# NVIDIA/flowtron

Hardware: AMD Instinct MI355X
Metric: mel-frames/sec training (2-flow, 80-mel) (higher is better)
Workload: dtype bf16; 1 GPU; BASELINE configs[1]: 2-flow LJS config.json model, per-GPU batch 32, T_max=862, L_max=157, attn-prior + CTC on, fwd+loss+bwd+clip+RAdam; global_batch=32, parallelism=dp1, mfma_operands=bf16, storage=fp32, skipped_steps=0

## Files before the change

flowtron_amd/_lib.py:

```python
from __future__ import annotations

import ctypes as C
import os

import torch

_HERE = os.path.dirname(os.path.abspath(__file__))
LIB_PATH = os.path.join(_HERE, "libflowtron_hip.so")

FT_F32, FT_BF16, FT_F16 = 0, 1, 2
GEMM_SPLITK = 1
GEMM_SPLITK_DET = 2
GEMM_C16 = 4
ACT_NONE, ACT_TANH, ACT_RELU, ACT_SIGMOID = 0, 1, 2, 3

_p, _i, _l, _f, _sz, _d = C.c_void_p, C.c_int, C.c_int64, C.c_float, C.c_size_t, C.c_double


class GemmArgs(C.Structure):
    _fields_ = [("A", _p), ("B", _p), ("C", _p), ("bias", _p),
                ("M", _i), ("N", _i), ("K", _i), ("batch", _i),
                ("sAm", _l), ("sAk", _l), ("sBk", _l), ("sBn", _l), ("ldc", _l),
                ("bsA", _l), ("bsB", _l), ("bsC", _l),
                ("alpha", _f), ("beta", _f), ("act", _i), ("mode", _i), ("flags", _i),
                ("work", _p), ("work_bytes", _sz)]


class GemmImgArgs(C.Structure):
    _fields_ = [("A", _p), ("B", _p), ("C", _p), ("bias", _p), ("M", _i), ("N", _i), ("K", _i),
                ("lda", _l), ("ldb", _l), ("ldc", _l), ("a_kmajor", _i), ("b_kmajor", _i),
                ("alpha", _f), ("beta", _f), ("act", _i), ("flags", _i),
                ("rowmap", _p), ("rows_dev", _p), ("compact", _i), ("k_shift", _i), ("r1_row", _p), ("r1_col", _p),
                ("split_work", _p), ("split_work_bytes", _sz), ("a_rows", _p)]


class GemmImgPlan(C.Structure):
    _fields_ = [(n, _i) for n in ("tile_rows", "stage_k", "gather", "atomics", "det", "splits", "chunk_w")]


class GemmImgGroupPlan(C.Structure):
    _fields_ = [(n, _i) for n in ("tile_rows", "splits", "ksteps", "atomics", "launch", "unit0", "tiles")]


GEMM_GROUP_MAX = 48


class LstmFwdRole(C.Structure):
    _fields_ = [("gx", _p), ("lens", _p), ("y", _p), ("ldy", _l), ("gates", _p), ("cell", _p), ("wimg", _p), ("state_h", _p), ("state_c", _p),
                ("B", C.c_int32), ("ldb", C.c_int32), ("t0", C.c_int32), ("t1", C.c_int32), ("gx16", C.c_int32)]


class LstmBwdRole(C.Structure):
# ... 34 lines not shown
STYLE_BATCH, STYLE_TIME_AND_BATCH = 0, 1

SIGNATURES = {
    "ft_abi_version": ([], _i),
    "ft_last_error": ([], C.c_char_p),
    "ft_debug_hold_cus": ([_i, _l, _p], _i),
    "ft_gemm": ([C.POINTER(GemmArgs), _p], _i),
    "ft_gemm_workspace_bytes": ([C.POINTER(GemmArgs)], _sz),
    "ft_bf16_image_bytes": ([_l, _l], _sz),
    "ft_bf16_image": ([_p, _l, _l, _l, _p, _p], _i),
    "ft_bf16_image_colsum": ([_p, _l, _l, _l, _p, _p, _p], _i),
    "ft_bf16_image_colsum_acc": ([_p, _l, _l, _l, _p, _p, _p], _i),
    "ft_gemm_img": ([C.POINTER(GemmImgArgs), _p], _i),
    "ft_gemm_img_split_work_bytes": ([_i, _i, _i], _sz),
    "ft_gemm_img_plan": ([C.POINTER(GemmImgArgs), C.POINTER(GemmImgPlan)], _i),
    "ft_gemm_img_group": ([C.POINTER(GemmImgArgs), _i, _p], _i),
    "ft_gemm_img_group_plan": ([C.POINTER(GemmImgArgs), _i, C.POINTER(GemmImgGroupPlan)], _i),
    "ft_bf16_image_split3": ([_p, _l, _l, _l, _p, _i, _p], _i),
    "ft_bf16_image_split3_im2col": ([_p, _p, _i, _i, _i, _i, _p, _p], _i),
    "ft_bf16_image_split3_im2col_f16": ([_p, _p, _i, _i, _i, _i, _p, _p], _i),
    "ft_bf16_image_table": ([C.POINTER(ImgDesc), _i, _p], _i),
    "ft_bf16_image_table_f16": ([C.POINTER(ImgDesc), _i, _p], _i),
    "ft_bf16_image_split3_f16": ([_p, _l, _l, _l, _p, _i, _p], _i),
    "ft_rowmap_build": ([_p, _p, _p, _i, _i, _p], _i),
    "ft_chunk_gather_rows": ([_p, _p, _p, _i, _i, _i, _i, _p], _i),
    "ft_bf16_image_rows": ([_p, _l, _l, _l, _p, _p, _p, _p, _p], _i),
    "ft_bf16_image_rows_acc": ([_p, _l, _l, _l, _p, _p, _p, _p, _p], _i),
    "ft_bf16_image_rows_into": ([_p, _l, _l, _l, _p, _l, _l, _l, _p, _p, _p], _i),
    "ft_img_gemv_rows": ([_p, _l, _i, _p, _p, _p, _l, _p, _p, _p, _i, _i, _p], _i),
    "ft_img_gemv_rows_bwd": ([_p, _l, _i, _p, _l, _p, _p, _p, _p, _l, _p], _i),
# ... 207 lines not shown
```

flowtron_amd/csrc/api.hip:

```cpp
#include "common.h"

thread_local char g_ft_err[512] = {0};

extern "C" int ft_abi_version(void) { return FT_ABI_VERSION; }
extern "C" const char* ft_last_error(void) { return g_ft_err; }

namespace {
__global__ __launch_bounds__(64) void hold_cus_k(long long ticks, int* sink) {
    extern __shared__ int big[];
    const long long t0 = wall_clock64();
    int n = 0;
    while (wall_clock64() - t0 < ticks) { big[threadIdx.x] = ++n; __builtin_amdgcn_s_sleep(64); }
    if (sink && big[threadIdx.x] == -1) sink[0] = n;
}
}
extern "C" int ft_debug_hold_cus(int n_wg, int64_t ticks, void* stream) {
    FT_CHECK_ARG(n_wg >= 1 && n_wg <= 256 && ticks >= 0);
    if (ticks > 500000000LL) ticks = 500000000LL;
    const int lds = 160 * 1024;
    FT_CHECK_HIP(hipFuncSetAttribute(reinterpret_cast<const void*>(hold_cus_k), hipFuncAttributeMaxDynamicSharedMemorySize, lds));
    hipLaunchKernelGGL(hold_cus_k, dim3(n_wg), dim3(64), lds, reinterpret_cast<hipStream_t>(stream), (long long)ticks, (int*)nullptr);
    FT_CHECK_LAUNCH();
    return FT_OK;
}
// ... 1 lines not shown
```

flowtron_amd/csrc/common.h:

```cpp
#pragma once
#include <hip/hip_runtime.h>
#include <stdint.h>
#include <stdio.h>
#include <stdarg.h>
#include "../../include/flowtron_hip.h"

extern thread_local char g_ft_err[512];

static inline int ft_fail(int code, const char* fmt, ...) {
    va_list ap;
    va_start(ap, fmt);
    vsnprintf(g_ft_err, sizeof(g_ft_err), fmt, ap);
    va_end(ap);
    return code;
}

#define FT_CHECK_ARG(cond)                                                            \
    do {                                                                              \
        if (!(cond)) return ft_fail(FT_EINVAL, "%s: invalid argument: %s", __func__, #cond); \
    } while (0)

#define FT_CHECK_LAUNCH()                                                             \
    do {                                                                              \
        hipError_t e_ = hipGetLastError();                                            \
// ... 137 lines not shown
```

flowtron_amd/csrc/gemm_bf16.hip:

```cpp
#include "common.h"
#include <stdlib.h>

namespace {

constexpr int TB = 128;

inline size_t up(size_t v, size_t m) { return (v + m - 1) / m * m; }

__device__ __forceinline__ uint4 pack8(const float (&v)[8]) {
    uint4 o;
    o.x = pack_op16x2(v[0], v[1]); o.y = pack_op16x2(v[2], v[3]);
    o.z = pack_op16x2(v[4], v[5]); o.w = pack_op16x2(v[6], v[7]);
    return o;
}

__device__ __forceinline__ int mapped_rows(const int* rdev, int Rp, int& Rz) {
    const int R = *rdev;
    const int z = (R + 32 + 255) & ~255;
    Rz = z < Rp ? z : Rp;
    return R;
}

__device__ __forceinline__ void img_rows_body(const float* __restrict__ src, long sr, long sc, int R, int Cc,
                                              unsigned short* __restrict__ dst, int Rp, int Cp, int vec,
// ... 182 lines not shown
}

struct BfP {
    const unsigned short* A; const unsigned short* B; float* C; const float* bias;
    int M, N, nk;
    long lda, ldb, ldc;
    float alpha, beta;
    int act, gx, gy, splits, ksteps;
    int vec_c;
    const int* rowmap; const int* rows_dev; int compact, k_shift;
    int chunk_w;
    const float* r1row; const float* r1col;
    long c_slice;
    int c16;
    const int* a_rows;
};

typedef __attribute__((address_space(3))) void lds_void;
typedef const __attribute__((address_space(1))) void glb_void;
typedef __attribute__((ext_vector_type(4))) short bf16x4;

template <bool KM, int RT = 128>
struct Operand {
    static constexpr int NS = RT / 64;
    static constexpr int WT = RT / 32;
    const unsigned short* src[NS];
    size_t kstride;
    int dst[NS];
    int roff;
    __device__ __forceinline__ void init(const unsigned short* img, long ld, int r0, int wave, int lane, int wsel) {
        const int li = lane & 15, kg = lane >> 4;
// ... 86 lines not shown
    }
    __device__ __forceinline__ void issue(unsigned char* sbuf, int t) const {
#pragma unroll
        for (int g = 0; g < NS; ++g) {
            if constexpr (GA)
                __builtin_amdgcn_global_load_lds((glb_void*)(srcg[g] + (size_t)t * 64), (lds_void*)(sbuf + dst0 + g * 1024), 16, 0, 0);
            else
                __builtin_amdgcn_global_load_lds((glb_void*)(src0 + (size_t)t * 64 + (size_t)g * ld8 + ((g & 1) ? xodd : 0)),
                                                 (lds_void*)(sbuf + dst0 + g * 1024), 16, 0, 0);
        }
    }
    __device__ __forceinline__ bf16x8 frag(const unsigned char* sbuf, int i, int ks) const {
        return *reinterpret_cast<const bf16x8*>(sbuf + ((roff + (i << 11)) ^ (ks << 6)));
    }
};

template <bool AKM, bool BKM, bool SPLIT, int RTA, int KS = 32, bool SB = false, bool GA = false>
__device__ __forceinline__ void gemm_bf16_body(const BfP& p, int tile, const int slice, const int nslices, const bool plain) {
    static_assert(!SB || (KS == 64 && RTA == 128 && !SPLIT), "single-buffer form: 128 x 128 x 64 store kernels");
    static_assert(!GA || (SB && !AKM), "row gather: the single-buffer form, k-contiguous A");
    constexpr int KQ = KS / 32;
    constexpr int OPA = RTA * 64 * KQ, OPB = 8192 * KQ;
    constexpr int TI = RTA / 32;
    __shared__ __attribute__((aligned(1024))) unsigned char smem[(SB ? 1 : 2) * (OPA + OPB)];
    const int tid = threadIdx.x, lane = tid & 63, wave = tid >> 6;
    const int wm = wave >> 1, wn = wave & 1;
    const int li = lane & 15, kg = lane >> 4;
    int t0 = slice * p.ksteps;
    int t1 = (t0 + p.ksteps < p.nk) ? t0 + p.ksteps : p.nk;
    int rows_lim = p.M, gy = p.gy;
// ... 2 lines not shown
        if (p.compact == 1) {
            rows_lim = R < p.M ? R : p.M;
            gy = (rows_lim + RTA - 1) / RTA;
            if (gy == 0) return;
        } else {
            int nk_eff = (R - p.k_shift + 31) >> 5;
            nk_eff = nk_eff < p.nk ? nk_eff : p.nk;
            if constexpr (SPLIT) {
                const int ks = (nk_eff + nslices - 1) / nslices;
                t0 = slice * ks;
                t1 = t0 + ks < nk_eff ? t0 + ks : nk_eff;
                if (t0 >= t1) return;
            } else t1 = t1 < nk_eff ? t1 : nk_eff;
        }
    }
    int mt, nt;
    if (p.chunk_w > 0 && gy >= 16) {
        const int xcd = tile & 7, idx = tile >> 3;
        const int qm = gy >> 3, rm = gy & 7;
        const int mh = qm + (xcd < rm ? 1 : 0);
        const int m_lo = xcd * qm + (xcd < rm ? xcd : rm);
        if (idx >= mh * p.gx) return;
        const int per_chunk = mh * p.chunk_w;
        const int ch = idx / per_chunk, within = idx - ch * per_chunk;
        const int left = p.gx - ch * p.chunk_w;
        const int cw = left < p.chunk_w ? left : p.chunk_w;
        const int mi = within / cw;
        mt = m_lo + mi;
        nt = ch * p.chunk_w + (within - mi * cw);
    } else {
        const int total = p.gx * gy, q = total >> 3, r = total & 7;
        const int xcd = tile & 7, idx = tile >> 3;
        if (tile >= total) return;
        tile = xcd * q + (xcd < r ? xcd : r) + idx;
        mt = tile / p.gx;
        nt = tile % p.gx;
    }
    const int m0 = mt * RTA, n0 = nt * TB;

    Operand<AKM, RTA> oa;
    Operand<BKM, 128> ob;
    Operand64<RTA, GA> oa64;
    Operand64<128> ob64;
    if constexpr (GA) oa64.init_rows(p.A, p.lda, m0, wave, lane, wm, p.a_rows, rows_lim - 1);
    else if constexpr (KS == 64 && !AKM) oa64.init(p.A, p.lda, m0, wave, lane, wm); else oa.init(p.A, p.lda, m0, wave, lane, wm);
    if constexpr (KS == 64 && !BKM) ob64.init(p.B, p.ldb, n0, wave, lane, wn); else ob.init(p.B, p.ldb, n0, wave, lane, wn);

    f32x4 acc[TI][4];
// ... 37 lines not shown
        }
        if constexpr (BKM) {
#pragma unroll
            for (int j = 0; j < 4; ++j) b[j] = __builtin_shufflevector(tb[2 * j], tb[2 * j + 1], 0, 1, 2, 3, 4, 5, 6, 7);
        }
    };
    auto multiply = [&](const bf16x8 (&a)[TI], const bf16x8 (&b)[4]) {
#pragma unroll
        for (int i = 0; i < TI; ++i)
#pragma unroll
            for (int j = 0; j < 4; ++j) {
                if constexpr (SPLIT) acc[i][j] = mfma16(a[i], b[j], acc[i][j]);
                else acc[i][j] = mfma16(b[j], a[i], acc[i][j]);
            }
    };
    const int s0 = t0 / KQ, s1 = (t1 + KQ - 1) / KQ;
    if (s0 < s1) issue_stage(smem, s0);
    if constexpr (SB) {
        for (int t = s0; t < s1; ++t) {
            asm volatile("s_waitcnt vmcnt(0)" ::: "memory");
            __syncthreads();
            bf16x8 a0[TI], b0[4], a1[TI], b1[4];
            load_frags(smem, 0, a0, b0);
            multiply(a0, b0);
            load_frags(smem, 1, a1, b1);
            __syncthreads();
            if (t + 1 < s1) issue_stage(smem, t + 1);
            multiply(a1, b1);
        }
    } else {
        for (int t = s0; t < s1; ++t) {
// ... 20 lines not shown
                if (p.compact == 1) { row = p.rowmap[row]; if (row < 0) continue; }
#pragma unroll
                for (int j = 0; j < 4; ++j) {
                    const int col = n0 + wn * 64 + j * 16 + li;
                    if (col >= p.N) continue;
                    float v = p.alpha * acc[i][j][r];
                    if (p.bias && slice == 0) v += p.bias[col];
                    float* cp = p.C + (long)row * p.ldc + col;
                    if (plain) *cp = p.beta != 0.f ? *cp + v : v;
                    else atomicAdd(cp, v);
                }
            }
        return;
    }

    const bool vec = p.vec_c != 0;
#pragma unroll
    for (int i = 0; i < TI; ++i) {
        int row = m0 + wm * (RTA / 2) + i * 16 + li;
        if (row >= rows_lim) continue;
        if (p.compact == 1) { row = p.rowmap[row]; if (row < 0) continue; }
#pragma unroll
        for (int j = 0; j < 4; ++j) {
            const int col = n0 + wn * 64 + j * 16 + kg * 4;
            if (col >= p.N) continue;
            float* cp = p.C + (size_t)slice * p.c_slice + (long)row * p.ldc + col;
            float v[4] = {p.alpha * acc[i][j][0], p.alpha * acc[i][j][1], p.alpha * acc[i][j][2], p.alpha * acc[i][j][3]};
            const int nv = (p.N - col < 4) ? p.N - col : 4;
            const bool full = vec && nv == 4;
            if (p.beta != 0.f) {
                if (full) { const float4 c = *reinterpret_cast<const float4*>(cp); v[0] += p.beta * c.x; v[1] += p.beta * c.y; v[2] += p.beta * c.z; v[3] += p.beta * c.w; }
                else for (int r = 0; r < nv; ++r) v[r] += p.beta * cp[r];
            }
            const float r1 = p.r1row ? p.r1row[row] : 0.f;
#pragma unroll
            for (int r = 0; r < 4; ++r) {
                if (r < nv && p.bias) v[r] += p.bias[col + r];
                if (r < nv && p.r1row) v[r] = fmaf(r1, p.r1col[col + r], v[r]);
                if (p.act == FT_ACT_TANH) v[r] = tanhf_(v[r]);
                else if (p.act == FT_ACT_RELU) v[r] = fmaxf(v[r], 0.f);
                else if (p.act == FT_ACT_SIGMOID) v[r] = sigmoidf_(v[r]);
            }
            if (p.c16) {
                unsigned short* hp = reinterpret_cast<unsigned short*>(p.C) + (long)row * p.ldc + col;
                if (full) *reinterpret_cast<uint2*>(hp) = make_uint2(pack_op16x2(v[0], v[1]), pack_op16x2(v[2], v[3]));
                else for (int r = 0; r < nv; ++r) hp[r] = f2op16(v[r]);
            } else if (full) *reinterpret_cast<float4*>(cp) = make_float4(v[0], v[1], v[2], v[3]);
            else for (int r = 0; r < nv; ++r) cp[r] = v[r];
        }
    }
}

template <bool AKM, bool BKM, bool SPLIT, int RTA, int KS = 32, bool SB = false, bool GA = false>
__global__ __launch_bounds__(256, SB ? 4 : (RTA == 256 || KS == 64) ? 2 : 4) void gemm_bf16_k(BfP p) {
    gemm_bf16_body<AKM, BKM, SPLIT, RTA, KS, SB, GA>(p, blockIdx.x, blockIdx.y, gridDim.y, false);
}

constexpr int GROUP_MAX = 48;
constexpr int GROUP_PLAIN = 1 << 8, GROUP_BETA1 = 1 << 9, GROUP_COMPACT = 1 << 10, GROUP_SHIFT = 12;
struct GroupTable {
    const unsigned short* A[GROUP_MAX]; const unsigned short* B[GROUP_MAX]; float* C[GROUP_MAX]; const float* bias[GROUP_MAX];
    const int* rows_dev[GROUP_MAX];
    float alpha[GROUP_MAX];
    int M[GROUP_MAX], N[GROUP_MAX], nk[GROUP_MAX], lda[GROUP_MAX], ldb[GROUP_MAX], ldc[GROUP_MAX];
    int how[GROUP_MAX];
// ... 10 lines not shown
        const int mid = (d + hi) >> 1;
        if (u >= t.unit0[mid]) d = mid; else hi = mid;
    }
    const int how = t.how[d], splits = how & 0xff;
    BfP p;
    p.A = t.A[d]; p.B = t.B[d]; p.C = t.C[d]; p.bias = t.bias[d];
    p.M = t.M[d]; p.N = t.N[d]; p.nk = t.nk[d];
    p.lda = t.lda[d]; p.ldb = t.ldb[d]; p.ldc = t.ldc[d];
    p.alpha = t.alpha[d]; p.beta = (how & GROUP_BETA1) ? 1.f : 0.f;
    p.act = FT_ACT_NONE;
    p.gx = (p.N + TB - 1) / TB; p.gy = (p.M + RTA - 1) / RTA;
    p.splits = splits; p.ksteps = (p.nk + splits - 1) / splits;
    p.vec_c = 0;
    p.rowmap = nullptr; p.rows_dev = t.rows_dev[d]; p.compact = (how & GROUP_COMPACT) ? 2 : 0; p.k_shift = how >> GROUP_SHIFT;
    p.chunk_w = 0; p.r1row = nullptr; p.r1col = nullptr; p.c_slice = 0; p.c16 = 0; p.a_rows = nullptr;
    const int local = u - t.unit0[d], tiles = p.gx * p.gy;
    const int slice = local / tiles;
    gemm_bf16_body<true, true, true, RTA>(p, local - slice * tiles, slice, splits, (how & GROUP_PLAIN) != 0);
}


struct KernelSel { int tile_rows, stage_k, gather, atomics; };

template <bool AKM, bool BKM>
void launch_s(const BfP& p, dim3 grid, const KernelSel& k, hipStream_t st) {
    if (k.tile_rows == 256) {
        if (k.atomics) hipLaunchKernelGGL((gemm_bf16_k<AKM, BKM, true, 256>), grid, dim3(256), 0, st, p);
        else hipLaunchKernelGGL((gemm_bf16_k<AKM, BKM, false, 256>), grid, dim3(256), 0, st, p);
    } else {
        if (k.atomics) hipLaunchKernelGGL((gemm_bf16_k<AKM, BKM, true, 128>), grid, dim3(256), 0, st, p);
        else if constexpr (!(AKM && BKM)) {
            if constexpr (!AKM) {
                if (k.gather) { hipLaunchKernelGGL((gemm_bf16_k<false, BKM, false, 128, 64, true, true>), grid, dim3(256), 0, st, p); return; }
            }
            if (k.stage_k == 64) hipLaunchKernelGGL((gemm_bf16_k<AKM, BKM, false, 128, 64, true>), grid, dim3(256), 0, st, p);
            else hipLaunchKernelGGL((gemm_bf16_k<AKM, BKM, false, 128>), grid, dim3(256), 0, st, p);
        } else hipLaunchKernelGGL((gemm_bf16_k<AKM, BKM, false, 128>), grid, dim3(256), 0, st, p);
    }
}

__global__ __launch_bounds__(256) void splitk_reduce_k(const float* __restrict__ work, int S, long MN, int N, float* __restrict__ C, long ldc,
                                                       const float* __restrict__ bias) {
    const long n4 = MN >> 2;
    for (long i = blockIdx.x * (long)blockDim.x + threadIdx.x; i < n4; i += (long)gridDim.x * blockDim.x) {
        const long e = i << 2;
        const long m = e / N;
        const int n = (int)(e - m * N);
        float4 a = *reinterpret_cast<const float4*>(work + e);
        for (int sl = 1; sl < S; ++sl) {
            const float4 b = *reinterpret_cast<const float4*>(work + (size_t)sl * MN + e);
            a.x += b.x; a.y += b.y; a.z += b.z; a.w += b.w;
        }
        if (bias) { a.x += bias[n]; a.y += bias[n + 1]; a.z += bias[n + 2]; a.w += bias[n + 3]; }
        *reinterpret_cast<float4*>(C + m * ldc + n) = a;
// ... 15 lines not shown
        const long smax = K / 512;
        if (s > smax) s = smax;
        if (s > 64) s = 64;
        if (s < 1) s = 1;
    }
    if (compact == 1) s = 1;
    *big_out = big;
    return s;
}

struct ImgPlan {
    bool big, wide, det_on;
    bool atomics;
    KernelSel sel;
    int gx, gy, ksteps, splits, chunk_w, gridx, vec_c, c16;
};
int plan_images(const float* C, long ldc, int a_km, int b_km, int M, int N, int K, float beta, int act, int flags, int compact, bool r1,
                const void* split_work, size_t split_work_bytes, bool a_rows, ImgPlan* pl) {
    pl->c16 = (flags & FT_GEMM_C16) ? 1 : 0;
    if (pl->c16 && (beta != 0.f || (flags & (FT_GEMM_SPLITK | FT_GEMM_SPLITK_DET))))
        return ft_fail(FT_EINVAL, "ft_gemm_img: FT_GEMM_C16 takes beta == 0 and no split-K");
    const bool det = (flags & FT_GEMM_SPLITK_DET) && split_work && act == FT_ACT_NONE && beta == 0.f && compact == 0 && !r1 && K >= 2048 &&
                     N % 4 == 0 && ldc % 4 == 0 && reinterpret_cast<uintptr_t>(C) % 16 == 0 && reinterpret_cast<uintptr_t>(split_work) % 16 == 0;
    const bool can_split = det || ((flags & FT_GEMM_SPLITK) && act == FT_ACT_NONE && (beta == 0.f || beta == 1.f) && K >= 2048 && !r1);
    bool big;
    long s = plan_slices(M, N, K, can_split, compact, &big);
    const int RTA = big ? 256 : TB;
    const int nk = cdiv(K, 32);
    pl->big = big;
    pl->gx = cdiv(N, TB); pl->gy = cdiv(M, RTA);
// ... 11 lines not shown
    if (a_rows && (!pl->wide || pl->splits != 1))
        return ft_fail(FT_EINVAL, "ft_gemm_img: a_rows is read by the 64-wide single-buffer kernel only (FT_GEMM_BF16_WIDE=0 / FT_GEMM_BF16_TILE=256 exclude it)");
    pl->det_on = det && pl->splits > 1;
    pl->atomics = pl->splits > 1 && !pl->det_on;
    pl->sel.tile_rows = big ? 256 : TB;
    pl->sel.atomics = pl->atomics ? 1 : 0;
    pl->sel.stage_k = (pl->wide && !pl->atomics) ? 64 : 32;
    pl->sel.gather = (a_rows && pl->sel.stage_k == 64) ? 1 : 0;
    static const int order_on = [] { const char* e = getenv("FT_GEMM_BF16_ORDER"); return e ? atoi(e) : 1; }();
    pl->chunk_w = 0;
    pl->gridx = pl->gx * pl->gy;
    if (order_on && pl->splits == 1 && pl->gy >= 16) {
        long cw = (2l << 20) / ((long)TB * (long)nk * 32 * 2);
        pl->chunk_w = (int)(cw < 1 ? 1 : (cw > pl->gx ? pl->gx : cw));
        pl->gridx = 8 * ((pl->gy + 7) / 8) * pl->gx;
    }
    return FT_OK;
}

int run_images(const unsigned short* A, long lda, int a_km, const unsigned short* B, long ldb, int b_km, float* C, long ldc,
               const float* bias, int M, int N, int K, float alpha, float beta, int act, int flags, hipStream_t st,
               const int* rowmap = nullptr, const int* rows_dev = nullptr, int compact = 0, int k_shift = 0,
               const float* r1row = nullptr, const float* r1col = nullptr, float* split_work = nullptr, size_t split_work_bytes = 0,
               const int* a_rows = nullptr) {
    ImgPlan pl;
    const int prc = plan_images(C, ldc, a_km, b_km, M, N, K, beta, act, flags, compact, r1row != nullptr, split_work, split_work_bytes,
                                a_rows != nullptr, &pl);
    if (prc != FT_OK) return prc;
    BfP p;
    p.a_rows = a_rows;
// ... 1 lines not shown
    p.M = M; p.N = N; p.nk = cdiv(K, 32); p.lda = lda; p.ldb = ldb; p.ldc = ldc;
    p.alpha = alpha; p.beta = beta; p.act = act;
    p.rowmap = rowmap; p.rows_dev = rows_dev; p.compact = compact; p.k_shift = k_shift;
    p.r1row = r1row; p.r1col = r1col;
    p.c_slice = 0;
    p.c16 = pl.c16;
    p.gx = pl.gx; p.gy = pl.gy; p.vec_c = pl.vec_c;
    p.ksteps = pl.ksteps; p.splits = pl.splits; p.chunk_w = pl.chunk_w;
    const bool det_on = pl.det_on;
    if (det_on) {
        p.C = split_work; p.ldc = N; p.c_slice = (long)M * N; p.bias = nullptr;
        p.vec_c = 1;
    } else if (p.splits > 1 && beta == 0.f) {
        FT_CHECK_HIP(hipMemset2DAsync(C, sizeof(float) * ldc, 0, sizeof(float) * N, M, st));
    }
    const dim3 grid(pl.gridx, p.splits);
    if (a_km) { if (b_km) launch_s<true, true>(p, grid, pl.sel, st); else launch_s<true, false>(p, grid, pl.sel, st); }
    else      { if (b_km) launch_s<false, true>(p, grid, pl.sel, st); else launch_s<false, false>(p, grid, pl.sel, st); }
    if (det_on) {
        const long n4 = ((long)M * N) >> 2;
        const int blocks = (int)((n4 + 255) / 256 < 4096 ? (n4 + 255) / 256 : 4096);
        hipLaunchKernelGGL(splitk_reduce_k, dim3(blocks), dim3(256), 0, st, split_work, p.splits, (long)M * N, N, C, ldc, bias);
    }
    FT_CHECK_LAUNCH();
    return FT_OK;
}

#define IMG_CHECK_ARG(cond)                                                           \
    do {                                                                              \
        if (!(cond)) return ft_fail(FT_EINVAL, "%s: invalid argument: %s", who, #cond); \
    } while (0)
// ... 344 lines not shown
    if (const int rc = check_img_args(a, __func__)) return rc;
    FT_CHECK_ARG(out != nullptr);
    ImgPlan pl;
    const int rc = plan_images(a->C, a->ldc, a->a_kmajor, a->b_kmajor, a->M, a->N, a->K, a->beta, a->act, a->flags, a->compact,
                               a->r1_row != nullptr, a->split_work, a->split_work_bytes, a->a_rows != nullptr, &pl);
    if (rc != FT_OK) return rc;
    out->tile_rows = pl.sel.tile_rows;
    out->stage_k = pl.sel.stage_k;
    out->gather = pl.sel.gather;
    out->atomics = pl.sel.atomics;
    out->det = pl.det_on ? 1 : 0;
    out->splits = pl.splits;
    out->chunk_w = pl.chunk_w;
    return FT_OK;
}
#endif

extern "C" int FT_OPNAME(ft_gemm_img)(const ft_gemm_img_args* a, void* stream) {
    if (const int rc = check_img_args(a, __func__)) return rc;
    return run_images(reinterpret_cast<const unsigned short*>(a->A), a->lda, a->a_kmajor, reinterpret_cast<const unsigned short*>(a->B),
                      a->ldb, a->b_kmajor, a->C, a->ldc, a->bias, a->M, a->N, a->K, a->alpha, a->beta, a->act, a->flags,
                      reinterpret_cast<hipStream_t>(stream), a->rowmap, a->rows_dev, a->compact, a->k_shift, a->r1_row, a->r1_col,
                      reinterpret_cast<float*>(a->split_work), a->split_work_bytes, a->a_rows);
}

#if FT_OPFMT == 0
extern "C" int ft_gemm_img_group_plan(const ft_gemm_img_args* probs, int n, ft_gemm_img_group_plan_t* out) {
    FT_CHECK_ARG(out != nullptr);
    GroupProb g[GROUP_MAX];
    int order[2][GROUP_MAX], cnt[2];
// ... 104 lines not shown
```

flowtron_amd/ops.py:

```python
from __future__ import annotations

import ctypes as C
from typing import List, Optional, Sequence

import torch

from . import _lib as L



def _c(t: torch.Tensor) -> torch.Tensor:
    return t if t.is_contiguous() else t.contiguous()


import os as _os
_BF16_IMAGES = True


def gemm_raw(A, B, Cm, M, N, K, sAm, sAk, sBk, sBn, ldc, bias=None, act=L.ACT_NONE, alpha=1.0, beta=0.0,
             batch=1, bsA=0, bsB=0, bsC=0, mode=None, splitk=False):
    L.require_cuda(A, B, Cm, bias)
    a = L.GemmArgs(L.ptr(A), L.ptr(B), L.ptr(Cm), L.ptr(bias), M, N, K, batch,
                   sAm, sAk, sBk, sBn, ldc, bsA, bsB, bsC, alpha, beta, act,
                   L.mfma_mode() if mode is None else mode, L.GEMM_SPLITK if splitk else 0,
# ... 200 lines not shown


_GX16 = True


def gx16_ok(mode, rowmap, T, B, H, reverse, xs, N, device):
    return (_GX16 and L.is16(mode) and rowmap is not None and not reverse and rowmap.T == T and rowmap.B == B and _PERSIST_IMG == "1"
            and linear_uses_images(mode, T * B, N, xs) and (len(xs) == 1 or _CAT_IMAGES)
            and B <= 32 and lstm_persistent(B, H, reverse, mode, device))


def images_apply(mode, M, N, K):
    return _BF16_IMAGES and L.is16(mode) and M >= 32 and N >= 32 and K >= 16 and M * N * K >= (1 << 20)


def _gemm_img_args(A, a_km, a_ptr, B, b_km, b_ptr, Cm, M, N, K, ldc, bias=None, act=L.ACT_NONE, alpha=1.0, beta=0.0, splitk=False,
                   rowmap=None, compact=0, k_shift=0, rank1=None, c16=False, a_rows=None, split_work_bytes=None):
    L.require_cuda(Cm, bias)
    flags, work, need = (L.GEMM_SPLITK if splitk else 0), None, 0
    if splitk == "det":
        need = L.lib().ft_gemm_img_split_work_bytes(M, N, K)
        if split_work_bytes is not None:
            need = min(need, int(split_work_bytes))
        flags = L.GEMM_SPLITK_DET if need else 0
        work = torch.empty(need, device=Cm.device, dtype=torch.uint8) if need else None
    if c16:
        assert Cm.dtype == op16_dtype(A.fmt) and not splitk and beta == 0.0
        flags |= L.GEMM_C16
    a = L.GemmImgArgs(a_ptr, b_ptr, L.ptr(Cm), L.ptr(bias), M, N, K, A.ld, B.ld, ldc, int(a_km), int(b_km),
                      alpha, beta, act, flags,
                      L.ptr(rowmap.map) if rowmap is not None else None, L.ptr(rowmap.rows) if rowmap is not None else None,
                      int(compact) if rowmap is not None else 0, int(k_shift),
                      L.ptr(rank1[0]) if rank1 is not None else None, rank1[1] if rank1 is not None else None,
                      L.ptr(work), need, L.ptr(a_rows) if a_rows is not None else None)
    assert A.fmt == B.fmt, "operand images of different formats"
    return a, work


def gemm_img(A, a_km, a_ptr, B, b_km, b_ptr, Cm, M, N, K, ldc, **kw):
    a, _work = _gemm_img_args(A, a_km, a_ptr, B, b_km, b_ptr, Cm, M, N, K, ldc, **kw)
# ... 61 lines not shown
    if leaf is None:
        return
    if id(leaf) in q["seen"]:
        flush_weight_grads()
    q["seen"][id(leaf)] = 0


def weight_grad_gemm(W, dW, A, a_ptr, B, b_ptr, Cm, M, N, K, ldc, **kw):
    if not _dw_deferrable(W, dW):
        gemm_img(A, 1, a_ptr, B, 1, b_ptr, Cm, M, N, K, ldc, splitk=True, **kw)
        return
    a, _work = _gemm_img_args(A, 1, a_ptr, B, 1, b_ptr, Cm, M, N, K, ldc, splitk=True, **kw)
    _DWQ["items"].append((a, A.fmt, L.stream(), Cm.device, (A.buf, B.buf, Cm.detach(), kw.get("rowmap"), kw.get("bias"))))
    if len(_DWQ["items"]) >= L.GEMM_GROUP_MAX:
        flush_weight_grads()


def gemm_img_group(arg_list, fmt, stream=None):
    arr = (L.GemmImgArgs * len(arg_list))(*arg_list)
    L.check(L.op16("ft_gemm_img_group", fmt)(arr, len(arg_list), L.stream() if stream is None else stream), "ft_gemm_img_group")


def gemm_img_group_plan(arg_list):
    arr = (L.GemmImgArgs * len(arg_list))(*arg_list)
    out = (L.GemmImgGroupPlan * len(arg_list))()
    L.check(L.lib().ft_gemm_img_group_plan(arr, len(arg_list), out), "ft_gemm_img_group_plan")
    return list(out)


def _dw_run(batch):
# ... 1989 lines not shown
```

include/flowtron_hip.h:

```cpp
#ifndef FLOWTRON_HIP_H
#define FLOWTRON_HIP_H

#include <stddef.h>
#include <stdint.h>

#ifdef __cplusplus
extern "C" {
#endif

#define FT_ABI_VERSION 15

enum { FT_OK = 0, FT_EINVAL = -1, FT_EHIP = -2, FT_EUNSUPPORTED = -3 };
enum { FT_F32 = 0, FT_BF16 = 1, FT_F16 = 2 };
enum { FT_ACT_NONE = 0, FT_ACT_TANH = 1, FT_ACT_RELU = 2, FT_ACT_SIGMOID = 3 };
enum { FT_GEMM_SPLITK = 1, FT_GEMM_SPLITK_DET = 2, FT_GEMM_C16 = 4 };

int ft_abi_version(void);
const char* ft_last_error(void);
int ft_debug_hold_cus(int n_wg, int64_t ticks, void* stream);

typedef struct {
    const float* A; const float* B; float* C; const float* bias;
    int M, N, K, batch;
    int64_t sAm, sAk, sBk, sBn, ldc;
// ... 13 lines not shown
    int64_t lda, ldb, ldc;
    int a_kmajor, b_kmajor;
    float alpha, beta;
    int act, flags;
    const int32_t* rowmap; const int32_t* rows_dev;
    int compact, k_shift;
    const float* r1_row; const float* r1_col;
    void* split_work; size_t split_work_bytes;
    const int32_t* a_rows;
} ft_gemm_img_args;
size_t ft_gemm_img_split_work_bytes(int M, int N, int K);
typedef struct { int tile_rows;
                 int stage_k;
                 int gather, atomics, det, splits, chunk_w; } ft_gemm_img_plan_t;
int ft_gemm_img_plan(const ft_gemm_img_args* a, ft_gemm_img_plan_t* out);
typedef struct { int tile_rows, splits, ksteps, atomics, launch, unit0, tiles; } ft_gemm_img_group_plan_t;
int ft_gemm_img_group_plan(const ft_gemm_img_args* probs, int n, ft_gemm_img_group_plan_t* out);
int ft_gemm_img_group(const ft_gemm_img_args* probs, int n, void* stream);
size_t ft_bf16_image_bytes(int64_t rows, int64_t cols);
int ft_bf16_image(const float* src, int64_t ld, int64_t rows, int64_t cols, void* dst, void* stream);
int ft_bf16_image_colsum(const float* src, int64_t ld, int64_t rows, int64_t cols, void* dst, float* colsum, void* stream);
int ft_gemm_img(const ft_gemm_img_args* a, void* stream);
int ft_bf16_image_colsum_acc(const float* src, int64_t ld, int64_t rows, int64_t cols, void* dst, float* colsum, void* stream);
int ft_bf16_image_rows_acc(const float* src, int64_t ld, int64_t cap_rows, int64_t cols, void* dst, float* colsum,
                           const int32_t* rowmap, const int32_t* rows_dev, void* stream);
int ft_bf16_image_rows_act_bwd_acc(const float* dy, int64_t ld, const float* y, int64_t ldy, int act, int64_t cap_rows, int64_t cols,
                                   void* dst, float* colsum, const int32_t* rowmap, const int32_t* rows_dev, void* stream);
int ft_bf16_image_colsum_acc_f16(const float* src, int64_t ld, int64_t rows, int64_t cols, void* dst, float* colsum, void* stream);
int ft_bf16_image_rows_acc_f16(const float* src, int64_t ld, int64_t cap_rows, int64_t cols, void* dst, float* colsum,
                               const int32_t* rowmap, const int32_t* rows_dev, void* stream);
// ... 420 lines not shown
```

Before: 732,800 mel-frames/s.

## Split K of last-wave GEMM tiles across helper workgroups to fill idle CUs

Adds a tail-split scheme to the bf16 image GEMM. When the final partial wave of output tiles would leave many occupancy slots idle, extra helper workgroups are launched, and each takes a slice of the K stages for one tail tile. Partial accumulators go to a workspace, a ticket counter picks the last arriver, and that workgroup reduces the partials and runs the shared epilogue. This trades extra workspace traffic, atomics and a larger grid for better CU utilisation on wave-quantised GEMMs. It is enabled by default through an env var and a per-device workspace.

```diff
diff --git a/flowtron_amd/_lib.py b/flowtron_amd/_lib.py
--- a/flowtron_amd/_lib.py
+++ b/flowtron_amd/_lib.py
@@ -36,6 +36,10 @@
 
 class GemmImgPlan(C.Structure):
     _fields_ = [(n, _i) for n in ("tile_rows", "stage_k", "gather", "atomics", "det", "splits", "chunk_w")]
+
+
+class GemmImgTailPlan(C.Structure):
+    _fields_ = [(n, _i) for n in ("may_split", "slots", "helpers", "s_max", "min_stages")]
 
 
 class GemmImgGroupPlan(C.Structure):
@@ -100,6 +104,9 @@
     "ft_gemm_img": ([C.POINTER(GemmImgArgs), _p], _i),
     "ft_gemm_img_split_work_bytes": ([_i, _i, _i], _sz),
     "ft_gemm_img_plan": ([C.POINTER(GemmImgArgs), C.POINTER(GemmImgPlan)], _i),
+    "ft_gemm_img_tail_plan": ([C.POINTER(GemmImgArgs), C.POINTER(GemmImgTailPlan)], _i),
+    "ft_gemm_tail_work_bytes": ([], _sz),
+    "ft_debug_gemm_tail": ([_i, _i, _i], _i),
     "ft_gemm_img_group": ([C.POINTER(GemmImgArgs), _i, _p], _i),
     "ft_gemm_img_group_plan": ([C.POINTER(GemmImgArgs), _i, C.POINTER(GemmImgGroupPlan)], _i),
     "ft_bf16_image_split3": ([_p, _l, _l, _l, _p, _i, _p], _i),
diff --git a/flowtron_amd/csrc/api.hip b/flowtron_amd/csrc/api.hip
--- a/flowtron_amd/csrc/api.hip
+++ b/flowtron_amd/csrc/api.hip
@@ -4,6 +4,13 @@
 
 extern "C" int ft_abi_version(void) { return FT_ABI_VERSION; }
 extern "C" const char* ft_last_error(void) { return g_ft_err; }
+
+int g_ft_tail_slots = 0, g_ft_tail_smax = 0, g_ft_tail_minst = 0;
+extern "C" int ft_debug_gemm_tail(int slots, int s_max, int min_stages) {
+    FT_CHECK_ARG(slots >= 0 && slots <= 4096 && slots % 8 == 0 && s_max >= 0 && s_max <= 64 && min_stages >= 0);
+    g_ft_tail_slots = slots; g_ft_tail_smax = s_max; g_ft_tail_minst = min_stages;
+    return FT_OK;
+}
 
 namespace {
 __global__ __launch_bounds__(64) void hold_cus_k(long long ticks, int* sink) {
diff --git a/flowtron_amd/csrc/common.h b/flowtron_amd/csrc/common.h
--- a/flowtron_amd/csrc/common.h
+++ b/flowtron_amd/csrc/common.h
@@ -6,6 +6,7 @@
 #include "../../include/flowtron_hip.h"
 
 extern thread_local char g_ft_err[512];
+extern int g_ft_tail_slots, g_ft_tail_smax, g_ft_tail_minst;
 
 static inline int ft_fail(int code, const char* fmt, ...) {
     va_list ap;
diff --git a/flowtron_amd/csrc/gemm_bf16.hip b/flowtron_amd/csrc/gemm_bf16.hip
--- a/flowtron_amd/csrc/gemm_bf16.hip
+++ b/flowtron_amd/csrc/gemm_bf16.hip
@@ -220,7 +220,37 @@
     long c_slice;
     int c16;
     const int* a_rows;
+    float* tail_ws; int* tail_cnt;
+    int slots, grid0, tail_smax, tail_minst;
 };
+
+__host__ __device__ inline int tail_rule(int live, int slots, int stages, int s_max, int min_stages, int& full, int& t) {
+    full = live / slots * slots;
+    t = live - full;
+    if (t * 8 < slots || t * 2 > slots) return 1;
+    int s = slots / t;
+    s = s < s_max ? s : s_max;
+    const int sk = stages / min_stages;
+    s = s < sk ? s : sk;
+    return s < 1 ? 1 : s;
+}
+
+__device__ __forceinline__ bool tail_role(const BfP& p, bool helper, int live, int slots, int stages, int base, int& idx, int& ts_n,
+                                          int& ts_i, int& ts_unit) {
+    int full, t;
+    const int s = tail_rule(live, slots, stages, p.tail_smax, p.tail_minst, full, t);
+    if (helper) {
+        if (s < 2) return false;
+        const int j = idx / (s - 1);
+        if (j >= t) return false;
+        ts_i = 1 + idx - j * (s - 1); ts_n = s; ts_unit = base + j * s;
+        idx = full + j;
+        return true;
+    }
+    if (idx >= live) return false;
+    if (s >= 2 && idx >= full) { ts_n = s; ts_i = 0; ts_unit = base + (idx - full) * s; }
+    return true;
+}
 
 typedef __attribute__((address_space(3))) void lds_void;
 typedef const __attribute__((address_space(1))) void glb_void;
@@ -337,6 +367,46 @@
         return *reinterpret_cast<const bf16x8*>(sbuf + ((roff + (i << 11)) ^ (ks << 6)));
     }
 };
+
+template <int TI>
+__device__ __forceinline__ void store_epilogue(const BfP& p, const f32x4 (&acc)[TI][4], int mrow0, int ncol0, int rows_lim, int li, int kg,
+                                               int slice) {
+    const bool vec = p.vec_c != 0;
+#pragma unroll
+    for (int i = 0; i < TI; ++i) {
+        int row = mrow0 + i * 16 + li;
+        if (row >= rows_lim) continue;
+        if (p.compact == 1) { row = p.rowmap[row]; if (row < 0) continue; }
+#pragma unroll
+        for (int j = 0; j < 4; ++j) {
+            const int col = ncol0 + j * 16 + kg * 4;
+            if (col >= p.N) continue;
+            float* cp = p.C + (size_t)slice * p.c_slice + (long)row * p.ldc + col;
+            float v[4] = {p.alpha * acc[i][j][0], p.alpha * acc[i][j][1], p.alpha * acc[i][j][2], p.alpha * acc[i][j][3]};
+            const int nv = (p.N - col < 4) ? p.N - col : 4;
+            const bool full = vec && nv == 4;
+            if (p.beta != 0.f) {
+                if (full) { const float4 c = *reinterpret_cast<const float4*>(cp); v[0] += p.beta * c.x; v[1] += p.beta * c.y; v[2] += p.beta * c.z; v[3] += p.beta * c.w; }
+                else for (int r = 0; r < nv; ++r) v[r] += p.beta * cp[r];
+            }
+            const float r1 = p.r1row ? p.r1row[row] : 0.f;
+#pragma unroll
+            for (int r = 0; r < 4; ++r) {
+                if (r < nv && p.bias) v[r] += p.bias[col + r];
+                if (r < nv && p.r1row) v[r] = fmaf(r1, p.r1col[col + r], v[r]);
+                if (p.act == FT_ACT_TANH) v[r] = tanhf_(v[r]);
+                else if (p.act == FT_ACT_RELU) v[r] = fmaxf(v[r], 0.f);
+                else if (p.act == FT_ACT_SIGMOID) v[r] = sigmoidf_(v[r]);
+            }
+            if (p.c16) {
+                unsigned short* hp = reinterpret_cast<unsigned short*>(p.C) + (long)row * p.ldc + col;
+                if (full) *reinterpret_cast<uint2*>(hp) = make_uint2(pack_op16x2(v[0], v[1]), pack_op16x2(v[2], v[3]));
+                else for (int r = 0; r < nv; ++r) hp[r] = f2op16(v[r]);
+            } else if (full) *reinterpret_cast<float4*>(cp) = make_float4(v[0], v[1], v[2], v[3]);
+            else for (int r = 0; r < nv; ++r) cp[r] = v[r];
+        }
+    }
+}
 
 template <bool AKM, bool BKM, bool SPLIT, int RTA, int KS = 32, bool SB = false, bool GA = false>
 __device__ __forceinline__ void gemm_bf16_body(const BfP& p, int tile, const int slice, const int nslices, const bool plain) {
@@ -369,13 +439,26 @@
             } else t1 = t1 < nk_eff ? t1 : nk_eff;
         }
     }
+    int s0 = t0 / KQ, s1 = (t1 + KQ - 1) / KQ;
+    int ts_n = 1, ts_i = 0, ts_unit = 0;
+    bool helper = false;
+    if constexpr (SB) {
+        if (p.tail_ws && tile >= p.grid0) { helper = true; tile -= p.grid0; }
+    }
+    auto resolve = [&](int live, int slots, int base, int& idx) -> bool {
+        if constexpr (SB) {
+            if (p.tail_ws) return tail_role(p, helper, live, slots, s1 - s0, base, idx, ts_n, ts_i, ts_unit);
+        }
+        return idx < live;
+    };
     int mt, nt;
     if (p.chunk_w > 0 && gy >= 16) {
-        const int xcd = tile & 7, idx = tile >> 3;
+        const int xcd = tile & 7;
+        int idx = tile >> 3;
         const int qm = gy >> 3, rm = gy & 7;
         const int mh = qm + (xcd < rm ? 1 : 0);
         const int m_lo = xcd * qm + (xcd < rm ? xcd : rm);
-        if (idx >= mh * p.gx) return;
+        if (!resolve(mh * p.gx, p.slots >> 3, xcd * (p.slots >> 3), idx)) return;
         const int per_chunk = mh * p.chunk_w;
         const int ch = idx / per_chunk, within = idx - ch * per_chunk;
         const int left = p.gx - ch * p.chunk_w;
@@ -385,8 +468,8 @@
         nt = ch * p.chunk_w + (within - mi * cw);
     } else {
         const int total = p.gx * gy, q = total >> 3, r = total & 7;
+        if (!resolve(total, p.slots, 0, tile)) return;
         const int xcd = tile & 7, idx = tile >> 3;
-        if (tile >= total) return;
         tile = xcd * q + (xcd < r ? xcd : r) + idx;
         mt = tile / p.gx;
         nt = tile % p.gx;
@@ -454,7 +537,13 @@
                 else acc[i][j] = mfma16(b[j], a[i], acc[i][j]);
             }
     };
-    const int s0 = t0 / KQ, s1 = (t1 + KQ - 1) / KQ;
+    if constexpr (SB) {
+        if (ts_n > 1) {
+            const int per = (s1 - s0) / ts_n;
+            s0 += ts_i * per;
+            if (ts_i + 1 < ts_n) s1 = s0 + per;
+        }
+    }
     if (s0 < s1) issue_stage(smem, s0);
     if constexpr (SB) {
         for (int t = s0; t < s1; ++t) {
@@ -505,41 +594,49 @@
         return;
     }
 
-    const bool vec = p.vec_c != 0;
-#pragma unroll
-    for (int i = 0; i < TI; ++i) {
-        int row = m0 + wm * (RTA / 2) + i * 16 + li;
-        if (row >= rows_lim) continue;
-        if (p.compact == 1) { row = p.rowmap[row]; if (row < 0) continue; }
-#pragma unroll
-        for (int j = 0; j < 4; ++j) {
-            const int col = n0 + wn * 64 + j * 16 + kg * 4;
-            if (col >= p.N) continue;
-            float* cp = p.C + (size_t)slice * p.c_slice + (long)row * p.ldc + col;
-            float v[4] = {p.alpha * acc[i][j][0], p.alpha * acc[i][j][1], p.alpha * acc[i][j][2], p.alpha * acc[i][j][3]};
-            const int nv = (p.N - col < 4) ? p.N - col : 4;
-            const bool full = vec && nv == 4;
-            if (p.beta != 0.f) {
-                if (full) { const float4 c = *reinterpret_cast<const float4*>(cp); v[0] += p.beta * c.x; v[1] += p.beta * c.y; v[2] += p.beta * c.z; v[3] += p.beta * c.w; }
-                else for (int r = 0; r < nv; ++r) v[r] += p.beta * cp[r];
-            }
-            const float r1 = p.r1row ? p.r1row[row] : 0.f;
-#pragma unroll
-            for (int r = 0; r < 4; ++r) {
-                if (r < nv && p.bias) v[r] += p.bias[col + r];
-                if (r < nv && p.r1row) v[r] = fmaf(r1, p.r1col[col + r], v[r]);
-                if (p.act == FT_ACT_TANH) v[r] = tanhf_(v[r]);
-                else if (p.act == FT_ACT_RELU) v[r] = fmaxf(v[r], 0.f);
-                else if (p.act == FT_ACT_SIGMOID) v[r] = sigmoidf_(v[r]);
-            }
-            if (p.c16) {
-                unsigned short* hp = reinterpret_cast<unsigned short*>(p.C) + (long)row * p.ldc + col;
-                if (full) *reinterpret_cast<uint2*>(hp) = make_uint2(pack_op16x2(v[0], v[1]), pack_op16x2(v[2], v[3]));
-                else for (int r = 0; r < nv; ++r) hp[r] = f2op16(v[r]);
-            } else if (full) *reinterpret_cast<float4*>(cp) = make_float4(v[0], v[1], v[2], v[3]);
-            else for (int r = 0; r < nv; ++r) cp[r] = v[r];
-        }
-    }
+    if constexpr (SB) {
+        if (ts_n > 1) {
+            constexpr int SLAB = TB * TB;
+            float* mine = p.tail_ws + (size_t)(ts_unit + ts_i) * SLAB + tid * 4;
+#pragma unroll
+            for (int i = 0; i < TI; ++i)
+#pragma unroll
+                for (int j = 0; j < 4; ++j) *reinterpret_cast<f32x4*>(mine + (i * 4 + j) * 1024) = acc[i][j];
+            asm volatile("s_waitcnt vmcnt(0)" ::: "memory");
+            __syncthreads();
+            if (tid == 0) {
+                __builtin_amdgcn_fence(__ATOMIC_RELEASE, "agent");
+                asm volatile("s_waitcnt vmcnt(0)" ::: "memory");
+                const int ticket = __hip_atomic_fetch_add(p.tail_cnt + ts_unit, 1, __ATOMIC_RELAXED, __HIP_MEMORY_SCOPE_AGENT);
+                *reinterpret_cast<volatile int*>(smem) = ticket;
+            }
+            __syncthreads();
+            if (*reinterpret_cast<volatile int*>(smem) != ts_n - 1) return;
+            if (tid == 0) {
+                __hip_atomic_store(p.tail_cnt + ts_unit, 0, __ATOMIC_RELAXED, __HIP_MEMORY_SCOPE_AGENT);
+                __builtin_amdgcn_fence(__ATOMIC_ACQUIRE, "agent");
+                asm volatile("s_waitcnt vmcnt(0)" ::: "memory");
+            }
+            __syncthreads();
+            const float* first = p.tail_ws + (size_t)ts_unit * SLAB + tid * 4;
+#pragma unroll
+            for (int h = 0; h < TI / 2; ++h) {
+                f32x4 v[8];
+#pragma unroll
+                for (int q = 0; q < 8; ++q) v[q] = *reinterpret_cast<const f32x4*>(first + (h * 8 + q) * 1024);
+                for (int sl = 1; sl < ts_n; ++sl) {
+                    f32x4 w[8];
+#pragma unroll
+                    for (int q = 0; q < 8; ++q) w[q] = *reinterpret_cast<const f32x4*>(first + (size_t)sl * SLAB + (h * 8 + q) * 1024);
+#pragma unroll
+                    for (int q = 0; q < 8; ++q) v[q] += w[q];
+                }
+#pragma unroll
+                for (int q = 0; q < 8; ++q) acc[2 * h + (q >> 2)][q & 3] = v[q];
+            }
+        }
+    }
+    store_epilogue<TI>(p, acc, m0 + wm * (RTA / 2), n0 + wn * 64, rows_lim, li, kg, slice);
 }
 
 template <bool AKM, bool BKM, bool SPLIT, int RTA, int KS = 32, bool SB = false, bool GA = false>
@@ -580,6 +677,7 @@
     p.vec_c = 0;
     p.rowmap = nullptr; p.rows_dev = t.rows_dev[d]; p.compact = (how & GROUP_COMPACT) ? 2 : 0; p.k_shift = how >> GROUP_SHIFT;
     p.chunk_w = 0; p.r1row = nullptr; p.r1col = nullptr; p.c_slice = 0; p.c16 = 0; p.a_rows = nullptr;
+    p.tail_ws = nullptr; p.tail_cnt = nullptr; p.slots = 0; p.grid0 = 0; p.tail_smax = 1; p.tail_minst = 1;
     const int local = u - t.unit0[d], tiles = p.gx * p.gy;
     const int slice = local / tiles;
     gemm_bf16_body<true, true, true, RTA>(p, local - slice * tiles, slice, splits, (how & GROUP_PLAIN) != 0);
@@ -604,6 +702,31 @@
         } else hipLaunchKernelGGL((gemm_bf16_k<AKM, BKM, false, 128>), grid, dim3(256), 0, st, p);
     }
 }
+
+template <bool AKM, bool BKM, bool GA>
+int occupancy_slots() {
+    int dev = 0, cus = 0, nb = 0;
+    if (hipGetDevice(&dev) == hipSuccess && hipDeviceGetAttribute(&cus, hipDeviceAttributeMultiprocessorCount, dev) == hipSuccess &&
+        hipOccupancyMaxActiveBlocksPerMultiprocessor(&nb, gemm_bf16_k<AKM, BKM, false, 128, 64, true, GA>, 256, 0) == hipSuccess && nb > 0 && cus > 0)
+        return nb * cus;
+    (void)hipGetLastError();
+    return -1;
+}
+int sb_slots(int a_km, int b_km, int gather) {
+    static int cache[2][2][2];
+    int& c = cache[a_km ? 1 : 0][b_km ? 1 : 0][gather ? 1 : 0];
+    if (c == 0) {
+        if (a_km) c = b_km ? -1 : occupancy_slots<true, false, false>();
+        else if (gather) c = b_km ? occupancy_slots<false, true, true>() : occupancy_slots<false, false, true>();
+        else c = b_km ? occupancy_slots<false, true, false>() : occupancy_slots<false, false, false>();
+    }
+    return c > 0 ? c : 0;
+}
+
+constexpr int TAIL_SLOTS_MAX = 4096;
+constexpr size_t TAIL_CNT_BYTES = TAIL_SLOTS_MAX * sizeof(int);
+constexpr size_t TAIL_SLAB_BYTES = (size_t)TB * TB * sizeof(float);
+constexpr int TAIL_S_MAX = 2, TAIL_MIN_STAGES = 32;
 
 __global__ __launch_bounds__(256) void splitk_reduce_k(const float* __restrict__ work, int S, long MN, int N, float* __restrict__ C, long ldc,
                                                        const float* __restrict__ bias) {
@@ -649,6 +772,8 @@
     bool atomics;
     KernelSel sel;
     int gx, gy, ksteps, splits, chunk_w, gridx, vec_c, c16;
+    bool tail;
+    int slots, grid_ext, tail_smax, tail_minst;
 };
 int plan_images(const float* C, long ldc, int a_km, int b_km, int M, int N, int K, float beta, int act, int flags, int compact, bool r1,
                 const void* split_work, size_t split_work_bytes, bool a_rows, ImgPlan* pl) {
@@ -690,6 +815,34 @@
         long cw = (2l << 20) / ((long)TB * (long)nk * 32 * 2);
         pl->chunk_w = (int)(cw < 1 ? 1 : (cw > pl->gx ? pl->gx : cw));
         pl->gridx = 8 * ((pl->gy + 7) / 8) * pl->gx;
+    }
+    pl->tail = false; pl->slots = 0; pl->grid_ext = 0;
+    pl->tail_smax = g_ft_tail_smax > 0 ? g_ft_tail_smax : TAIL_S_MAX;
+    pl->tail_minst = g_ft_tail_minst > 0 ? g_ft_tail_minst : TAIL_MIN_STAGES;
+    const char* tail_env = getenv("FT_GEMM_TAIL_SPLIT");
+    if ((!tail_env || atoi(tail_env) != 0) && split_work && !(flags & (FT_GEMM_SPLITK | FT_GEMM_SPLITK_DET)) && pl->sel.stage_k == 64 &&
+        pl->splits == 1 && compact != 2) {
+        int slots = g_ft_tail_slots > 0 ? g_ft_tail_slots : sb_slots(a_km, b_km, pl->sel.gather);
+        slots = (slots < TAIL_SLOTS_MAX ? slots : TAIL_SLOTS_MAX) & ~7;
+        const int stages = nk / 2;
+        if (slots >= 8 && stages / pl->tail_minst >= 2) {
+            if (reinterpret_cast<uintptr_t>(split_work) % 16 != 0 || split_work_bytes < TAIL_CNT_BYTES + (size_t)slots * TAIL_SLAB_BYTES)
+                return ft_fail(FT_EINVAL, "ft_gemm_img: the tail-split workspace must be 16-byte aligned and hold %zu bytes (%d slots)",
+                               TAIL_CNT_BYTES + (size_t)slots * TAIL_SLAB_BYTES, slots);
+            int ext = 0, full, t;
+            if (compact == 1) ext = slots;
+            else if (pl->chunk_w > 0) {
+                for (int x = 0; x < 8; ++x) {
+                    const int mh = pl->gy / 8 + (x < pl->gy % 8 ? 1 : 0);
+                    const int sx = tail_rule(mh * pl->gx, slots / 8, stages, pl->tail_smax, pl->tail_minst, full, t);
+                    if (8 * t * (sx - 1) > ext) ext = 8 * t * (sx - 1);
+                }
+            } else {
+                const int sp = tail_rule(pl->gx * pl->gy, slots, stages, pl->tail_smax, pl->tail_minst, full, t);
+                ext = t * (sp - 1);
+            }
+            if (ext > 0) { pl->tail = true; pl->slots = slots; pl->grid_ext = ext; }
+        }
     }
     return FT_OK;
 }
@@ -721,7 +874,13 @@
     } else if (p.splits > 1 && beta == 0.f) {
         FT_CHECK_HIP(hipMemset2DAsync(C, sizeof(float) * ldc, 0, sizeof(float) * N, M, st));
     }
-    const dim3 grid(pl.gridx, p.splits);
+    p.tail_ws = nullptr; p.tail_cnt = nullptr; p.slots = 0; p.grid0 = pl.gridx; p.tail_smax = pl.tail_smax; p.tail_minst = pl.tail_minst;
+    if (pl.tail) {
+        p.tail_cnt = reinterpret_cast<int*>(split_work);
+        p.tail_ws = reinterpret_cast<float*>(reinterpret_cast<char*>(split_work) + TAIL_CNT_BYTES);
+        p.slots = pl.slots;
+    }
+    const dim3 grid(pl.gridx + pl.grid_ext, p.splits);
     if (a_km) { if (b_km) launch_s<true, true>(p, grid, pl.sel, st); else launch_s<true, false>(p, grid, pl.sel, st); }
     else      { if (b_km) launch_s<false, true>(p, grid, pl.sel, st); else launch_s<false, false>(p, grid, pl.sel, st); }
     if (det_on) {
@@ -1096,6 +1255,28 @@
     out->chunk_w = pl.chunk_w;
     return FT_OK;
 }
+
+extern "C" size_t ft_gemm_tail_work_bytes(void) {
+    int slots = g_ft_tail_slots;
+    for (int i = 0; i < 8; ++i) { const int s = sb_slots(i & 1, (i >> 1) & 1, (i >> 2) & 1); if (s > slots) slots = s; }
+    if (slots > TAIL_SLOTS_MAX) slots = TAIL_SLOTS_MAX;
+    return slots > 0 ? TAIL_CNT_BYTES + (size_t)slots * TAIL_SLAB_BYTES : 0;
+}
+
+extern "C" int ft_gemm_img_tail_plan(const ft_gemm_img_args* a, ft_gemm_img_tail_plan_t* out) {
+    if (const int rc = check_img_args(a, __func__)) return rc;
+    FT_CHECK_ARG(out != nullptr);
+    ImgPlan pl;
+    const int rc = plan_images(a->C, a->ldc, a->a_kmajor, a->b_kmajor, a->M, a->N, a->K, a->beta, a->act, a->flags, a->compact,
+                               a->r1_row != nullptr, a->split_work, a->split_work_bytes, a->a_rows != nullptr, &pl);
+    if (rc != FT_OK) return rc;
+    out->may_split = pl.tail ? 1 : 0;
+    out->slots = pl.slots;
+    out->helpers = pl.grid_ext;
+    out->s_max = pl.tail_smax;
+    out->min_stages = pl.tail_minst;
+    return FT_OK;
+}
 #endif
 
 extern "C" int FT_OPNAME(ft_gemm_img)(const ft_gemm_img_args* a, void* stream) {
diff --git a/flowtron_amd/ops.py b/flowtron_amd/ops.py
--- a/flowtron_amd/ops.py
+++ b/flowtron_amd/ops.py
@@ -238,6 +238,21 @@
     return _BF16_IMAGES and L.is16(mode) and M >= 32 and N >= 32 and K >= 16 and M * N * K >= (1 << 20)
 
 
+_TAIL_SPLIT = True
+_TAIL_WORK = {}
+
+
+def tail_workspace(device):
+    key = (device.index if device.index is not None else torch.cuda.current_device(), L.stream())
+    w = _TAIL_WORK.get(key)
+    if w is None:
+        with torch.cuda.device(key[0]):
+            need = L.lib().ft_gemm_tail_work_bytes()
+        w = torch.zeros(need, device=device, dtype=torch.uint8) if need else False
+        _TAIL_WORK[key] = w
+    return None if w is False else w
+
+
 def _gemm_img_args(A, a_km, a_ptr, B, b_km, b_ptr, Cm, M, N, K, ldc, bias=None, act=L.ACT_NONE, alpha=1.0, beta=0.0, splitk=False,
                    rowmap=None, compact=0, k_shift=0, rank1=None, c16=False, a_rows=None, split_work_bytes=None):
     L.require_cuda(Cm, bias)
@@ -248,6 +263,9 @@
             need = min(need, int(split_work_bytes))
         flags = L.GEMM_SPLITK_DET if need else 0
         work = torch.empty(need, device=Cm.device, dtype=torch.uint8) if need else None
+    elif not splitk and _TAIL_SPLIT and compact != 2:
+        work = tail_workspace(Cm.device)
+        need = work.numel() if work is not None else 0
     if c16:
         assert Cm.dtype == op16_dtype(A.fmt) and not splitk and beta == 0.0
         flags |= L.GEMM_C16
@@ -339,6 +357,13 @@
     _DWQ["items"].append((a, A.fmt, L.stream(), Cm.device, (A.buf, B.buf, Cm.detach(), kw.get("rowmap"), kw.get("bias"))))
     if len(_DWQ["items"]) >= L.GEMM_GROUP_MAX:
         flush_weight_grads()
+
+
+def gemm_img_tail_plan(A, a_km, a_ptr, B, b_km, b_ptr, Cm, M, N, K, ldc, **kw):
+    a, _work = _gemm_img_args(A, a_km, a_ptr, B, b_km, b_ptr, Cm, M, N, K, ldc, **kw)
+    plan = L.GemmImgTailPlan()
+    L.check(L.lib().ft_gemm_img_tail_plan(C.byref(a), C.byref(plan)), "ft_gemm_img_tail_plan")
+    return plan
 
 
 def gemm_img_group(arg_list, fmt, stream=None):
diff --git a/include/flowtron_hip.h b/include/flowtron_hip.h
--- a/include/flowtron_hip.h
+++ b/include/flowtron_hip.h
@@ -51,6 +51,10 @@
                  int stage_k;
                  int gather, atomics, det, splits, chunk_w; } ft_gemm_img_plan_t;
 int ft_gemm_img_plan(const ft_gemm_img_args* a, ft_gemm_img_plan_t* out);
+typedef struct { int may_split, slots, helpers, s_max, min_stages; } ft_gemm_img_tail_plan_t;
+int ft_gemm_img_tail_plan(const ft_gemm_img_args* a, ft_gemm_img_tail_plan_t* out);
+size_t ft_gemm_tail_work_bytes(void);
+int ft_debug_gemm_tail(int slots, int s_max, int min_stages);
 typedef struct { int tile_rows, splits, ksteps, atomics, launch, unit0, tiles; } ft_gemm_img_group_plan_t;
 int ft_gemm_img_group_plan(const ft_gemm_img_args* probs, int n, ft_gemm_img_group_plan_t* out);
 int ft_gemm_img_group(const ft_gemm_img_args* probs, int n, void* stream);
```

Result: no change. 731,600 mel-frames/s (-0.2%).
